# awkrail/svpc

Measured on AMD Instinct MI355X. Metric: train steps/sec (vivt, batch=16, clip_seq=12), higher is better.
Workload: dtype bf16x3; 1 GPU; MODEL_TYPE=vivt train step: N=16 videos/GPU x S=12 clips x Lv=100 frames x F=3072, Lt=22, D=768, H=12, L=6 (enc+step-enc+dec), V=951, A=384, E=10; dropout .1/.1/.4; fwd+bwd+allreduce+clip+BertAdam; mode=bf16x3, global_batch=16, parallelism=dp1, launch=hipGraph replay, gpus_requested=1

## Files before the change

svpc_amd/csrc/optimizer.hip:

```cpp
#include "common.h"

struct TensorMeta { float* p; float* g; float* m; float* v; float* ema; long long n; float wd; int pad; __bf16* shadow; __bf16* shadow_lo; };

constexpr int OPT_CHUNK = 16384;

__global__ __launch_bounds__(256) void opt_sumsq_kernel(const TensorMeta* __restrict__ meta, const int* __restrict__ chunk_tid,
                                                        const long long* __restrict__ chunk_start, float* __restrict__ partial) {
    __shared__ float red[4];
    const int c = blockIdx.x;
    const TensorMeta t = meta[chunk_tid[c]];
    const long long s = chunk_start[c];
    const long long e = s + OPT_CHUNK < t.n ? s + OPT_CHUNK : t.n;
    float acc = 0.f;
    if ((e - s) == OPT_CHUNK && ((((unsigned long long)(t.g + s)) & 15ull) == 0)) {
        const float4* g4 = reinterpret_cast<const float4*>(t.g + s);
        float4 v[OPT_CHUNK / 4 / 256];
#pragma unroll
        for (int k = 0; k < OPT_CHUNK / 4 / 256; ++k) v[k] = g4[threadIdx.x + 256 * k];
#pragma unroll
        for (int k = 0; k < OPT_CHUNK / 4 / 256; ++k) acc += v[k].x * v[k].x + v[k].y * v[k].y + v[k].z * v[k].z + v[k].w * v[k].w;
    } else {
        for (long long i = s + threadIdx.x; i < e; i += 256) { const float g = t.g[i]; acc += g * g; }
    }
    acc = block_sum_256(acc, red);
    if (threadIdx.x == 0) partial[c] = acc;
}
__global__ __launch_bounds__(256) void opt_norms_kernel(const float* __restrict__ partial, const int* __restrict__ tensor_chunk_off,
                                                        int n_tensors, float* __restrict__ norms_sq) {
    __shared__ float red[4];
    float tot = 0.f;
    for (int t = threadIdx.x; t < n_tensors; t += 256) {
        float s = 0.f;
        for (int c = tensor_chunk_off[t]; c < tensor_chunk_off[t + 1]; ++c) s += partial[c];
        norms_sq[t] = s;
        tot += s;
    }
    tot = block_sum_256(tot, red);
    if (threadIdx.x == 0) norms_sq[n_tensors] = tot;
}
__global__ __launch_bounds__(256) void opt_adam_kernel(const TensorMeta* __restrict__ meta, const int* __restrict__ chunk_tid,
                                                       const long long* __restrict__ chunk_start, const float* __restrict__ norms_sq,
                                                       int n_tensors, const float* __restrict__ hyper) {
    const int c = blockIdx.x;
    const int tid = chunk_tid[c];
    const TensorMeta t = meta[tid];
    const float lr = hyper[0], ema_decay = hyper[1], max_g = hyper[2], max_t = hyper[3], b1 = hyper[4], b2 = hyper[5], eps = hyper[6];
    float coef = 1.0f;
    if (max_g > 0.f) coef = fminf(1.0f, max_g / (sqrtf(norms_sq[n_tensors]) + 1e-6f));
    if (max_t > 0.f) {
        const float tn = sqrtf(norms_sq[tid]) * coef;
        coef *= fminf(1.0f, max_t / (tn + 1e-6f));
    }
    const long long s = chunk_start[c];
    const long long e = s + OPT_CHUNK < t.n ? s + OPT_CHUNK : t.n;
    const bool use_ema = t.ema && ema_decay >= 0.f;
    const unsigned long long al = (unsigned long long)(t.g + s) | (unsigned long long)(t.m + s) | (unsigned long long)(t.v + s) |
                                  (unsigned long long)(t.p + s) | (use_ema ? (unsigned long long)(t.ema + s) : 0ull) |
                                  ((t.shadow ? (unsigned long long)(t.shadow + s) : 0ull) << 1) |
                                  ((t.shadow && t.shadow_lo ? (unsigned long long)(t.shadow_lo + s) : 0ull) << 1);
    if ((e - s) == OPT_CHUNK && (al & 15ull) == 0) {
        constexpr int NB = 4, PER = OPT_CHUNK / 4 / 256 / NB;
        float4* __restrict__ g4 = reinterpret_cast<float4*>(t.g + s);
        float4* __restrict__ m4 = reinterpret_cast<float4*>(t.m + s);
        float4* __restrict__ v4 = reinterpret_cast<float4*>(t.v + s);
        float4* __restrict__ p4 = reinterpret_cast<float4*>(t.p + s);
        float4* __restrict__ e4 = reinterpret_cast<float4*>(t.ema + s);
        uint2* __restrict__ sh = reinterpret_cast<uint2*>(t.shadow + s);
        uint2* __restrict__ sl = reinterpret_cast<uint2*>(t.shadow_lo + s);
        for (int b = 0; b < NB; ++b) {
            float4 g[PER], m[PER], v[PER], p[PER], em[PER];
#pragma unroll
            for (int k = 0; k < PER; ++k) {
                const int i = threadIdx.x + 256 * (b * PER + k);
                g[k] = g4[i]; m[k] = m4[i]; v[k] = v4[i]; p[k] = p4[i];
                if (use_ema) em[k] = e4[i];
            }
#pragma unroll
            for (int k = 0; k < PER; ++k) {
                const int i = threadIdx.x + 256 * (b * PER + k);
                float gg[4] = {g[k].x, g[k].y, g[k].z, g[k].w}, mm[4] = {m[k].x, m[k].y, m[k].z, m[k].w};
                float vv[4] = {v[k].x, v[k].y, v[k].z, v[k].w}, pp[4] = {p[k].x, p[k].y, p[k].z, p[k].w};
                float ee[4] = {0.f, 0.f, 0.f, 0.f};
                if (use_ema) { ee[0] = em[k].x; ee[1] = em[k].y; ee[2] = em[k].z; ee[3] = em[k].w; }
                __bf16 hi[4], lo[4];
#pragma unroll
                for (int j = 0; j < 4; ++j) {
                    const float gj = gg[j] * coef;
                    mm[j] = b1 * mm[j] + (1.f - b1) * gj;
                    vv[j] = b2 * vv[j] + (1.f - b2) * gj * gj;
                    float upd = mm[j] / (sqrtf(vv[j]) + eps);
                    if (t.wd > 0.f) upd += t.wd * pp[j];
                    pp[j] -= lr * upd;
                    hi[j] = (__bf16)pp[j];
                    lo[j] = (__bf16)(pp[j] - (float)hi[j]);
                    if (use_ema) ee[j] = (1.f - ema_decay) * pp[j] + ema_decay * ee[j];
                }
                m4[i] = make_float4(mm[0], mm[1], mm[2], mm[3]);
                v4[i] = make_float4(vv[0], vv[1], vv[2], vv[3]);
                p4[i] = make_float4(pp[0], pp[1], pp[2], pp[3]);
                if (t.shadow) {
                    union { __bf16 h[4]; uint2 u; } ph, pl;
#pragma unroll
                    for (int j = 0; j < 4; ++j) { ph.h[j] = hi[j]; pl.h[j] = lo[j]; }
                    sh[i] = ph.u;
                    if (t.shadow_lo) sl[i] = pl.u;
                }
                if (use_ema) e4[i] = make_float4(ee[0], ee[1], ee[2], ee[3]);
            }
        }
        return;
    }
    for (long long i = s + threadIdx.x; i < e; i += 256) {
        const float g = t.g[i] * coef;
        const float m = b1 * t.m[i] + (1.f - b1) * g;
        const float v = b2 * t.v[i] + (1.f - b2) * g * g;
        float p = t.p[i];
        float upd = m / (sqrtf(v) + eps);
        if (t.wd > 0.f) upd += t.wd * p;
        p -= lr * upd;
        t.m[i] = m; t.v[i] = v; t.p[i] = p;
        if (t.shadow) {
            const __bf16 ph = (__bf16)p;
            t.shadow[i] = ph;
            if (t.shadow_lo) t.shadow_lo[i] = (__bf16)(p - (float)ph);
        }
        if (t.ema && ema_decay >= 0.f) t.ema[i] = (1.f - ema_decay) * p + ema_decay * t.ema[i];
    }
}
__global__ __launch_bounds__(256) void opt_zero_kernel(const TensorMeta* __restrict__ meta, const int* __restrict__ chunk_tid,
                                                       const long long* __restrict__ chunk_start) {
    const int c = blockIdx.x;
    const TensorMeta t = meta[chunk_tid[c]];
    const long long s = chunk_start[c];
    const long long e = s + OPT_CHUNK < t.n ? s + OPT_CHUNK : t.n;
    for (long long i = s + threadIdx.x; i < e; i += 256) t.g[i] = 0.f;
}

extern "C" {

int svpc_opt_chunk(void) { return OPT_CHUNK; }
int svpc_opt_meta_bytes(void) { return (int)sizeof(TensorMeta); }

int svpc_opt_step(const void* meta, const int* chunk_tid, const long long* chunk_start, const int* tensor_chunk_off, int n_tensors,
                  int n_chunks, float* partial, float* norms_sq, const float* hyper, hipStream_t s) {
    if (n_chunks == 0) return 0;
    hipLaunchKernelGGL(opt_sumsq_kernel, dim3(n_chunks), dim3(256), 0, s, (const TensorMeta*)meta, chunk_tid, chunk_start, partial);
    int rc = svpc_check_launch("opt_sumsq");
    if (rc) return rc;
    hipLaunchKernelGGL(opt_norms_kernel, dim3(1), dim3(256), 0, s, partial, tensor_chunk_off, n_tensors, norms_sq);
    rc = svpc_check_launch("opt_norms");
    if (rc) return rc;
    hipLaunchKernelGGL(opt_adam_kernel, dim3(n_chunks), dim3(256), 0, s, (const TensorMeta*)meta, chunk_tid, chunk_start, norms_sq,
                       n_tensors, hyper);
    return svpc_check_launch("opt_adam");
}
int svpc_opt_zero_grad(const void* meta, const int* chunk_tid, const long long* chunk_start, int n_chunks, hipStream_t s) {
    if (n_chunks == 0) return 0;
    hipLaunchKernelGGL(opt_zero_kernel, dim3(n_chunks), dim3(256), 0, s, (const TensorMeta*)meta, chunk_tid, chunk_start);
    return svpc_check_launch("opt_zero");
}

}
```

Baseline: 90.85 steps/s (one step = 16 clip-sequences per GPU; whole-job aggregate).

## Stage optimizer partials in LDS, reverse Adam chunk order, use nontemporal accesses

The norms kernel now copies all per-chunk partial sums into shared memory before the per-tensor reduction, so the strided serial global reads become LDS reads. The Adam kernel walks chunks in reverse block order, likely so it touches the most recently written gradients (still in cache from the sumsq pass) first. It also uses nontemporal loads and stores for the streaming m, v, g, param, shadow and EMA arrays, with explicit FMA and fp-contract off to keep the arithmetic well-defined. The optimizer is a small part of the step, and nontemporal hints could bypass cache lines that the following zero-grad or forward pass would have reused.

```diff
diff --git a/svpc_amd/csrc/optimizer.hip b/svpc_amd/csrc/optimizer.hip
--- a/svpc_amd/csrc/optimizer.hip
+++ b/svpc_amd/csrc/optimizer.hip
@@ -25,23 +25,95 @@
     acc = block_sum_256(acc, red);
     if (threadIdx.x == 0) partial[c] = acc;
 }
+constexpr int OPT_NORMS_STAGE = 12288;
 __global__ __launch_bounds__(256) void opt_norms_kernel(const float* __restrict__ partial, const int* __restrict__ tensor_chunk_off,
                                                         int n_tensors, float* __restrict__ norms_sq) {
     __shared__ float red[4];
+    __shared__ float stage[OPT_NORMS_STAGE];
+    const int n_chunks = tensor_chunk_off[n_tensors];
+    const bool staged = n_chunks <= OPT_NORMS_STAGE;
+    if (staged) {
+        for (int c = threadIdx.x; c < n_chunks; c += 256) stage[c] = partial[c];
+        __syncthreads();
+    }
     float tot = 0.f;
     for (int t = threadIdx.x; t < n_tensors; t += 256) {
         float s = 0.f;
-        for (int c = tensor_chunk_off[t]; c < tensor_chunk_off[t + 1]; ++c) s += partial[c];
+        if (staged) for (int c = tensor_chunk_off[t]; c < tensor_chunk_off[t + 1]; ++c) s += stage[c];
+        else for (int c = tensor_chunk_off[t]; c < tensor_chunk_off[t + 1]; ++c) s += partial[c];
         norms_sq[t] = s;
         tot += s;
     }
     tot = block_sum_256(tot, red);
     if (threadIdx.x == 0) norms_sq[n_tensors] = tot;
 }
+typedef float opt_f4 __attribute__((ext_vector_type(4)));
+typedef unsigned opt_u2 __attribute__((ext_vector_type(2)));
+typedef opt_f4 __attribute__((address_space(1))) * opt_f4p;
+typedef opt_u2 __attribute__((address_space(1))) * opt_u2p;
+struct AdamHyper { float wd, coef, lr, ema_decay, b1, b2, eps; };
+__device__ __forceinline__ void adam_elem(const AdamHyper& h, float g, float& m, float& v, float& p) {
+#pragma clang fp contract(off)
+    const float gj = g * h.coef;
+    m = __builtin_fmaf(h.b1, m, (1.f - h.b1) * gj);
+    v = __builtin_fmaf(h.b2, v, ((1.f - h.b2) * gj) * gj);
+    float upd = m / (sqrtf(v) + h.eps);
+    if (h.wd > 0.f) upd = __builtin_fmaf(h.wd, p, upd);
+    p = __builtin_fmaf(-h.lr, upd, p);
+}
+__device__ __forceinline__ float adam_ema(const AdamHyper& h, float p, float e) {
+#pragma clang fp contract(off)
+    return __builtin_fmaf(h.ema_decay, e, (1.f - h.ema_decay) * p);
+}
+constexpr int ADAM_PER = 4, ADAM_NB = OPT_CHUNK / 4 / 256 / ADAM_PER;
+struct AdamBatch { opt_f4 g[ADAM_PER], m[ADAM_PER], v[ADAM_PER], p[ADAM_PER], e[ADAM_PER]; };
+struct AdamChunk {
+    opt_f4p g, m, v, p, e; opt_u2p sh, sl;
+    bool use_ema, has_sh, has_sl;
+    AdamHyper h;
+};
+__device__ __forceinline__ void adam_load(const AdamChunk& k, AdamBatch& r, int b) {
+#pragma unroll
+    for (int q = 0; q < ADAM_PER; ++q) {
+        const int i = threadIdx.x + 256 * (b * ADAM_PER + q);
+        r.g[q] = __builtin_nontemporal_load(k.g + i); r.m[q] = __builtin_nontemporal_load(k.m + i);
+        r.v[q] = __builtin_nontemporal_load(k.v + i); r.p[q] = k.p[i];
+        if (k.use_ema) r.e[q] = k.e[i];
+    }
+}
+__device__ __forceinline__ void adam_apply(const AdamChunk& k, const AdamBatch& r, int b) {
+#pragma unroll
+    for (int q = 0; q < ADAM_PER; ++q) {
+        const int i = threadIdx.x + 256 * (b * ADAM_PER + q);
+        opt_f4 mm = r.m[q], vv = r.v[q], pp = r.p[q], ee = {0.f, 0.f, 0.f, 0.f};
+        if (k.use_ema) ee = r.e[q];
+        __bf16 hi[4], lo[4];
+#pragma unroll
+        for (int j = 0; j < 4; ++j) {
+            float m = mm[j], v = vv[j], p = pp[j];
+            adam_elem(k.h, r.g[q][j], m, v, p);
+            mm[j] = m; vv[j] = v; pp[j] = p;
+            hi[j] = (__bf16)p;
+            lo[j] = (__bf16)(p - (float)hi[j]);
+            if (k.use_ema) ee[j] = adam_ema(k.h, p, ee[j]);
+        }
+        __builtin_nontemporal_store(mm, k.m + i);
+        __builtin_nontemporal_store(vv, k.v + i);
+        __builtin_nontemporal_store(pp, k.p + i);
+        if (k.has_sh) {
+            union { __bf16 h[4]; opt_u2 u; } ph, pl;
+#pragma unroll
+            for (int j = 0; j < 4; ++j) { ph.h[j] = hi[j]; pl.h[j] = lo[j]; }
+            __builtin_nontemporal_store(ph.u, k.sh + i);
+            if (k.has_sl) __builtin_nontemporal_store(pl.u, k.sl + i);
+        }
+        if (k.use_ema) __builtin_nontemporal_store(ee, k.e + i);
+    }
+}
 __global__ __launch_bounds__(256) void opt_adam_kernel(const TensorMeta* __restrict__ meta, const int* __restrict__ chunk_tid,
                                                        const long long* __restrict__ chunk_start, const float* __restrict__ norms_sq,
                                                        int n_tensors, const float* __restrict__ hyper) {
-    const int c = blockIdx.x;
+    const int c = (int)(gridDim.x - 1 - blockIdx.x);
     const int tid = chunk_tid[c];
     const TensorMeta t = meta[tid];
     const float lr = hyper[0], ema_decay = hyper[1], max_g = hyper[2], max_t = hyper[3], b1 = hyper[4], b2 = hyper[5], eps = hyper[6];
@@ -54,77 +126,33 @@
     const long long s = chunk_start[c];
     const long long e = s + OPT_CHUNK < t.n ? s + OPT_CHUNK : t.n;
     const bool use_ema = t.ema && ema_decay >= 0.f;
+    const AdamHyper hy = {t.wd, coef, lr, ema_decay, b1, b2, eps};
     const unsigned long long al = (unsigned long long)(t.g + s) | (unsigned long long)(t.m + s) | (unsigned long long)(t.v + s) |
                                   (unsigned long long)(t.p + s) | (use_ema ? (unsigned long long)(t.ema + s) : 0ull) |
                                   ((t.shadow ? (unsigned long long)(t.shadow + s) : 0ull) << 1) |
                                   ((t.shadow && t.shadow_lo ? (unsigned long long)(t.shadow_lo + s) : 0ull) << 1);
     if ((e - s) == OPT_CHUNK && (al & 15ull) == 0) {
-        constexpr int NB = 4, PER = OPT_CHUNK / 4 / 256 / NB;
-        float4* __restrict__ g4 = reinterpret_cast<float4*>(t.g + s);
-        float4* __restrict__ m4 = reinterpret_cast<float4*>(t.m + s);
-        float4* __restrict__ v4 = reinterpret_cast<float4*>(t.v + s);
-        float4* __restrict__ p4 = reinterpret_cast<float4*>(t.p + s);
-        float4* __restrict__ e4 = reinterpret_cast<float4*>(t.ema + s);
-        uint2* __restrict__ sh = reinterpret_cast<uint2*>(t.shadow + s);
-        uint2* __restrict__ sl = reinterpret_cast<uint2*>(t.shadow_lo + s);
-        for (int b = 0; b < NB; ++b) {
-            float4 g[PER], m[PER], v[PER], p[PER], em[PER];
+        const AdamChunk k = {(opt_f4p)(t.g + s), (opt_f4p)(t.m + s), (opt_f4p)(t.v + s), (opt_f4p)(t.p + s), (opt_f4p)(t.ema + s),
+                             (opt_u2p)(t.shadow + s), (opt_u2p)(t.shadow_lo + s), use_ema, t.shadow != nullptr,
+                             t.shadow != nullptr && t.shadow_lo != nullptr, hy};
 #pragma unroll
-            for (int k = 0; k < PER; ++k) {
-                const int i = threadIdx.x + 256 * (b * PER + k);
-                g[k] = g4[i]; m[k] = m4[i]; v[k] = v4[i]; p[k] = p4[i];
-                if (use_ema) em[k] = e4[i];
-            }
-#pragma unroll
-            for (int k = 0; k < PER; ++k) {
-                const int i = threadIdx.x + 256 * (b * PER + k);
-                float gg[4] = {g[k].x, g[k].y, g[k].z, g[k].w}, mm[4] = {m[k].x, m[k].y, m[k].z, m[k].w};
-                float vv[4] = {v[k].x, v[k].y, v[k].z, v[k].w}, pp[4] = {p[k].x, p[k].y, p[k].z, p[k].w};
-                float ee[4] = {0.f, 0.f, 0.f, 0.f};
-                if (use_ema) { ee[0] = em[k].x; ee[1] = em[k].y; ee[2] = em[k].z; ee[3] = em[k].w; }
-                __bf16 hi[4], lo[4];
-#pragma unroll
-                for (int j = 0; j < 4; ++j) {
-                    const float gj = gg[j] * coef;
-                    mm[j] = b1 * mm[j] + (1.f - b1) * gj;
-                    vv[j] = b2 * vv[j] + (1.f - b2) * gj * gj;
-                    float upd = mm[j] / (sqrtf(vv[j]) + eps);
-                    if (t.wd > 0.f) upd += t.wd * pp[j];
-                    pp[j] -= lr * upd;
-                    hi[j] = (__bf16)pp[j];
-                    lo[j] = (__bf16)(pp[j] - (float)hi[j]);
-                    if (use_ema) ee[j] = (1.f - ema_decay) * pp[j] + ema_decay * ee[j];
-                }
-                m4[i] = make_float4(mm[0], mm[1], mm[2], mm[3]);
-                v4[i] = make_float4(vv[0], vv[1], vv[2], vv[3]);
-                p4[i] = make_float4(pp[0], pp[1], pp[2], pp[3]);
-                if (t.shadow) {
-                    union { __bf16 h[4]; uint2 u; } ph, pl;
-#pragma unroll
-                    for (int j = 0; j < 4; ++j) { ph.h[j] = hi[j]; pl.h[j] = lo[j]; }
-                    sh[i] = ph.u;
-                    if (t.shadow_lo) sl[i] = pl.u;
-                }
-                if (use_ema) e4[i] = make_float4(ee[0], ee[1], ee[2], ee[3]);
-            }
+        for (int b = 0; b < ADAM_NB; ++b) {
+            AdamBatch r;
+            adam_load(k, r, b);
+            adam_apply(k, r, b);
         }
         return;
     }
     for (long long i = s + threadIdx.x; i < e; i += 256) {
-        const float g = t.g[i] * coef;
-        const float m = b1 * t.m[i] + (1.f - b1) * g;
-        const float v = b2 * t.v[i] + (1.f - b2) * g * g;
-        float p = t.p[i];
-        float upd = m / (sqrtf(v) + eps);
-        if (t.wd > 0.f) upd += t.wd * p;
-        p -= lr * upd;
+        float m = t.m[i], v = t.v[i], p = t.p[i];
+        adam_elem(hy, t.g[i], m, v, p);
         t.m[i] = m; t.v[i] = v; t.p[i] = p;
         if (t.shadow) {
             const __bf16 ph = (__bf16)p;
             t.shadow[i] = ph;
             if (t.shadow_lo) t.shadow_lo[i] = (__bf16)(p - (float)ph);
         }
-        if (t.ema && ema_decay >= 0.f) t.ema[i] = (1.f - ema_decay) * p + ema_decay * t.ema[i];
+        if (use_ema) t.ema[i] = adam_ema(hy, p, t.ema[i]);
     }
 }
 __global__ __launch_bounds__(256) void opt_zero_kernel(const TensorMeta* __restrict__ meta, const int* __restrict__ chunk_tid,
```

Result: no change. 91.21 steps/s (one step = 16 clip-sequences per GPU; whole-job aggregate), median of 6 (+0.4%).
